# NetManAIOps/ChatTS

Hardware: NVIDIA H100
Metric: decode_tokens_per_s (higher is better)
Workload: dtype bf16

## Files before the change

chatts_b200/_cabi.py:

```python
import ctypes as C
import os

import torch

_HERE = os.path.dirname(os.path.abspath(__file__))
LIB_PATH = os.path.join(_HERE, "lib", "libchatts_b200.so")

OK = 0
BF16, F16 = 0, 1
EPI_NONE, EPI_GELU, EPI_SWIGLU, EPI_PARTIAL_F32, EPI_RESIDUAL, EPI_SPLITK_F32, EPI_SWIGLU_IL = 0, 1, 2, 3, 4, 5, 6

SYMBOLS = [
    "cts_version", "cts_arch", "cts_ctx_create", "cts_ctx_destroy", "cts_last_error",
    "cts_ts_patch_count", "cts_ts_patchify", "cts_gemm", "cts_gemm_suggest_split",
    "cts_reduce_bias_act", "cts_reduce_residual_rmsnorm", "cts_reduce_swiglu", "cts_qkv_rope_cache",
    "cts_embed_gather", "cts_attn_prefill", "cts_attn_decode_workspace_floats", "cts_attn_decode",
    "cts_greedy_advance", "cts_ipc_alloc", "cts_ipc_open", "cts_ipc_close", "cts_ipc_free",
    "cts_peer_allreduce_residual_rmsnorm", "cts_peer_greedy_advance", "cts_decode_chain",
    "cts_attn_prefill_lse", "cts_attn_bwd", "cts_swiglu", "cts_swiglu_bwd", "cts_rmsnorm_bwd", "cts_qkv_rope_bwd",
    "cts_ce_loss_grad", "cts_gather_rows", "cts_lora_wgrad", "cts_adamw", "cts_grad_norm_ws_floats", "cts_grad_norm_clip",
    "cts_lora_pack",
    "cts_sample_advance", "cts_rmsnorm", "cts_lm_head", "cts_decoder_step_ws_floats", "cts_decoder_step", "cts_ts_encode", "cts_gemm_decode_fused",
    "cts_peer_ll_region_bytes", "cts_peer_allreduce_ll", "cts_trace_enable", "cts_ts_encode_fused_ok", "cts_ts_encode_fused",
    "cts_rep_penalty_mark", "cts_rep_penalty_apply", "cts_gemm_w4", "cts_gemm_w4_suggest_split", "cts_gemm_w4_mma", "cts_gemm_w4_mma_suggest_split",
]
FUSED_RESIDUAL, FUSED_SWIGLU, FUSED_QKV_ROPE = 0, 1, 2
PACK_DESC_LONGS = 12


class CtsError(RuntimeError):
    pass


class GemmArgs(C.Structure):
    _fields_ = [
        ("w", C.c_void_p), ("w2", C.c_void_p), ("x", C.c_void_p), ("bias", C.c_void_p),
        ("residual", C.c_void_p), ("out", C.c_void_p), ("row_map", C.c_void_p),
        ("n", C.c_longlong), ("k", C.c_longlong), ("t", C.c_longlong),
        ("w_ld", C.c_longlong), ("x_ld", C.c_longlong), ("out_ld", C.c_longlong),
        ("dtype", C.c_int), ("epilogue", C.c_int), ("split_k", C.c_int), ("reserved", C.c_int),
        ("splitk_ws", C.c_void_p), ("tile_counters", C.c_void_p),
        ("next_w", C.c_void_p), ("next_n", C.c_longlong), ("next_k", C.c_longlong), ("next_ld", C.c_longlong),
        ("next_split", C.c_int), ("next_reserved", C.c_int), ("next_prefetch_bytes", C.c_longlong),
    ]


class ChainArgs(C.Structure):
    _fields_ = (
        [(k, C.c_int) for k in ("t", "hidden", "inter", "nh", "nkv", "head_dim", "phase_begin", "phase_end", "norm5_has_partial",
                                "dtype")] + [("split", C.c_int * 4)] +
        [(k, C.c_void_p) for k in ("wo", "wgu", "wd", "wqkv", "ao", "h", "xn", "act", "ln_post", "ln_next")] + [("eps", C.c_float)] +
        [(k, C.c_void_p) for k in ("bqkv", "q_norm_w", "k_norm_w", "positions", "cos_tab", "sin_tab", "slot_map", "q_out", "k_cache",
                                   "v_cache")] + [("page_size", C.c_int)] + [(k, C.c_void_p) for k in ("ws", "ssq", "sync")])


class LayerWeights(C.Structure):
    _fields_ = [(k, C.c_void_p) for k in ("wqkv", "bqkv", "q_norm", "k_norm", "wo", "wgu", "wd", "ln1", "ln2", "k_cache", "v_cache")]
# ... 70 lines not shown
    lib.cts_reduce_residual_rmsnorm.argtypes = [vp, vp, i, vp, vp, vp, f, vp, ll, ll, i, vp]
    lib.cts_reduce_swiglu.argtypes = [vp, vp, i, ll, ll, vp, i, i, vp]
    lib.cts_qkv_rope_cache.argtypes = [vp, vp, i, i, vp, vp, vp, vp, vp, vp, vp, vp, vp, vp, ll, i, i, i, i, vp, vp, f, i, vp]
    lib.cts_embed_gather.argtypes = [vp, vp, vp, vp, ll, ll, ll, i, vp]
    lib.cts_attn_prefill.argtypes = [vp, vp, vp, vp, vp, i, i, ll, i, i, i, f, vp, i, vp]
    lib.cts_attn_decode_workspace_floats.argtypes = [i, i, i, i]
    lib.cts_attn_decode_workspace_floats.restype = ll
    lib.cts_attn_decode.argtypes = [vp, vp, vp, vp, i, vp, i, vp, i, i, i, i, i, f, i, vp, vp, i, vp]
    lib.cts_greedy_advance.argtypes = [vp, vp, ll, i, vp, i, vp, vp, vp, vp, vp, vp, i, i, i, vp]
    lib.cts_ipc_alloc.argtypes = [vp, ll, C.POINTER(vp), C.c_char_p]
    lib.cts_ipc_open.argtypes = [vp, C.c_char_p, C.POINTER(vp)]
    lib.cts_ipc_close.argtypes = [vp, vp]
    lib.cts_ipc_free.argtypes = [vp, vp]
    lib.cts_peer_allreduce_residual_rmsnorm.argtypes = [vp, vp, i, vp, vp, vp, i, i, i, vp, vp, vp, f, vp, ll, ll, i, vp]
    lib.cts_peer_ll_region_bytes.argtypes = [i, i, ll]
    lib.cts_peer_ll_region_bytes.restype = ll
    lib.cts_peer_allreduce_ll.argtypes = [vp, vp, i, vp, ll, vp, i, i, i, vp, vp, vp, f, vp, ll, ll, i, vp]
    lib.cts_peer_allreduce_ll.restype = i
    lib.cts_trace_enable.argtypes = [vp, vp]
    lib.cts_gemm_w4.argtypes = [vp, C.POINTER(GemmW4Args), vp]
    lib.cts_gemm_w4_suggest_split.argtypes = [vp, ll, ll]
    lib.cts_gemm_w4_mma.argtypes = [vp, C.POINTER(GemmW4fArgs), vp]
    lib.cts_gemm_w4_mma_suggest_split.argtypes = [vp, ll, ll, ll]
    lib.cts_rep_penalty_mark.argtypes = [vp, vp, vp, i, vp, i, ll, vp]
    lib.cts_rep_penalty_apply.argtypes = [vp, vp, ll, ll, i, vp, i, f, i, vp]
    lib.cts_ts_encode_fused_ok.argtypes = [C.POINTER(TsEncodeArgs)]
    lib.cts_ts_encode_fused.argtypes = [vp, C.POINTER(TsEncodeArgs), vp]
    lib.cts_decode_chain.argtypes = [vp, C.POINTER(ChainArgs), vp]
    lib.cts_decode_chain.restype = i
    lib.cts_peer_greedy_advance.argtypes = [vp, vp, ll, i, i, i, vp, vp, vp, i, vp, i, vp, vp, vp, vp, vp, vp, i, i, i, vp]
    lib.cts_peer_greedy_advance.restype = i
    lib.cts_gemm_decode_fused.argtypes = [vp, C.POINTER(FusedGemmArgs), vp]
    lib.cts_gemm_decode_fused.restype = i
    lib.cts_ts_encode.argtypes = [vp, C.POINTER(TsEncodeArgs), vp]
    lib.cts_ts_encode.restype = i
    lib.cts_rmsnorm.argtypes = [vp, vp, vp, f, vp, ll, ll, i, vp]
    lib.cts_lm_head.argtypes = [vp, vp, vp, vp, ll, ll, ll, i, vp]
    lib.cts_decoder_step_ws_floats.argtypes = [C.POINTER(DecoderStepArgs)]
    lib.cts_decoder_step_ws_floats.restype = ll
    lib.cts_decoder_step.argtypes = [vp, C.POINTER(DecoderStepArgs), vp]
    for name in ("cts_rmsnorm", "cts_lm_head", "cts_decoder_step"):
        getattr(lib, name).restype = i
    lib.cts_sample_advance.argtypes = [vp, vp, ll, i, f, i, f, C.c_ulonglong, vp, i, vp, vp, vp, vp, vp, vp, i, i, i, vp]
    lib.cts_sample_advance.restype = i
    lib.cts_attn_prefill_lse.argtypes = [vp, vp, vp, vp, vp, i, i, ll, i, i, i, f, vp, vp, i, vp]
    lib.cts_attn_bwd.argtypes = [vp, vp, vp, vp, vp, vp, vp, vp, i, i, ll, i, i, i, f, vp, vp, vp, vp, i, vp]
    lib.cts_swiglu.argtypes = [vp, vp, ll, ll, i, vp, i, vp]
    lib.cts_swiglu_bwd.argtypes = [vp, vp, vp, ll, ll, i, vp, i, vp]
    lib.cts_rmsnorm_bwd.argtypes = [vp, vp, vp, vp, f, vp, vp, ll, ll, i, vp]
    lib.cts_qkv_rope_bwd.argtypes = [vp, vp, vp, vp, vp, vp, vp, vp, vp, vp, f, vp, ll, i, i, i, i, vp]
    lib.cts_ce_loss_grad.argtypes = [vp, vp, ll, vp, ll, ll, f, vp, vp, i, i, vp]
    lib.cts_gather_rows.argtypes = [vp, vp, vp, ll, ll, vp, i, vp]
    lib.cts_lora_wgrad.argtypes = [vp, vp, ll, ll, i, ll, vp, ll, ll, i, ll, f, vp, ll, ll, i, vp]
    lib.cts_adamw.argtypes = [vp, vp, vp, vp, vp, ll, f, f, f, f, f, i, vp, vp]
    lib.cts_grad_norm_ws_floats.argtypes = []
    lib.cts_grad_norm_ws_floats.restype = ll
    lib.cts_grad_norm_clip.argtypes = [vp, vp, ll, f, vp, vp, vp]
    lib.cts_lora_pack.argtypes = [vp, vp, vp, i, ll, vp, i, vp]
    for name in ("cts_attn_prefill_lse", "cts_attn_bwd", "cts_swiglu", "cts_swiglu_bwd", "cts_rmsnorm_bwd", "cts_qkv_rope_bwd",
                 "cts_ce_loss_grad", "cts_gather_rows", "cts_lora_wgrad", "cts_adamw", "cts_grad_norm_clip", "cts_lora_pack"):
        getattr(lib, name).restype = i
    for name in ("cts_ipc_alloc", "cts_ipc_open", "cts_ipc_close", "cts_ipc_free", "cts_peer_allreduce_residual_rmsnorm"):
        getattr(lib, name).restype = i
    for name in ("cts_ts_patch_count", "cts_ts_patchify", "cts_gemm", "cts_gemm_suggest_split", "cts_reduce_bias_act",
                 "cts_reduce_residual_rmsnorm", "cts_reduce_swiglu", "cts_qkv_rope_cache", "cts_embed_gather",
                 "cts_attn_prefill", "cts_attn_decode", "cts_greedy_advance", "cts_ctx_create"):
# ... 60 lines not shown
        self._trace = buf
        return buf

    def trace_end(self):
        torch.cuda.synchronize()
        self.lib.cts_trace_enable(self.h, None)
        buf, self._trace = self._trace, None
        n = min(int(buf[0]), int(buf[1]))
        return buf[2: 2 + 2 * n].view(n, 2).cpu().numpy()

    def ts_patch_count(self, x, num_features, patch_size):
        n = x.shape[0]
        row_len = x.numel() // max(n, 1)
        dev = x.device
        valid = torch.empty(n, dtype=torch.int32, device=dev)
        cnt = torch.empty(n, dtype=torch.int32, device=dev)
        off = torch.empty(n + 1, dtype=torch.int32, device=dev)
        mx = torch.empty(1, dtype=torch.int32, device=dev)
        self._chk(self.lib.cts_ts_patch_count(self.h, _p(x), dtype_code(x.dtype), n, row_len, num_features, patch_size,
                                              _p(valid), _p(cnt), _p(off), _p(mx), _stream()), 2)
        return valid, cnt, off, mx

    def ts_patchify(self, x, num_features, patch_size, mode, pos_table, emb_dim, max_seq_len, valid, off, mx,
                    max_patches, rows_out):
        n = x.shape[0]
        row_len = x.numel() // max(n, 1)
        self._chk(self.lib.cts_ts_patchify(self.h, _p(x), dtype_code(x.dtype), n, row_len, num_features, patch_size, mode,
                                           _p(pos_table), emb_dim, max_seq_len, _p(valid), _p(off), _p(mx), max_patches,
                                           _p(rows_out), rows_out.shape[1], _stream()))

    def suggest_split(self, n, k, t, dual=False):
        return int(self.lib.cts_gemm_suggest_split(self.h, n, k, t, int(dual)))

    def gemm(self, x, w, out, *, w2=None, bias=None, residual=None, row_map=None, epilogue=EPI_NONE, split_k=1, t=None,
             splitk_ws=None, tile_counters=None, next_w=None, next_split=1, next_bytes=0):
        a = GemmArgs()
        if next_w is not None and next_bytes > 0:
            a.next_w, a.next_n, a.next_k, a.next_ld = next_w.data_ptr(), next_w.shape[0], next_w.shape[1], next_w.stride(0)
            a.next_split, a.next_prefetch_bytes = int(next_split), int(next_bytes)
        a.w, a.w2, a.x = w.data_ptr(), (w2.data_ptr() if w2 is not None else None), x.data_ptr()
        a.bias = bias.data_ptr() if bias is not None else None
        a.residual = residual.data_ptr() if residual is not None else None
        a.out = out.data_ptr()
        a.row_map = row_map.data_ptr() if row_map is not None else None
        a.n, a.k = w.shape[0], w.shape[1]
        a.t = x.shape[0] if t is None else t
        a.w_ld, a.x_ld = w.stride(0), x.stride(0)
        a.out_ld = out.stride(-2) if epilogue not in (EPI_PARTIAL_F32, EPI_SPLITK_F32) else a.n
        a.splitk_ws = splitk_ws.data_ptr() if splitk_ws is not None else None
        a.tile_counters = tile_counters.data_ptr() if tile_counters is not None else None
        a.dtype, a.epilogue, a.split_k = dtype_code(x.dtype), epilogue, split_k
        self._chk(self.lib.cts_gemm(self.h, C.byref(a), _stream()))

    def gemm_w4(self, x, qw, scales, zeros, group_size, out, split_k, t=None):
        a = GemmW4Args()
        a.qw, a.scales, a.zeros, a.x, a.out = qw.data_ptr(), scales.data_ptr(), zeros.data_ptr(), x.data_ptr(), out.data_ptr()
        a.n, a.k = qw.shape[0], qw.shape[1] * 2
        a.t = x.shape[0] if t is None else t
        a.x_ld, a.group_size, a.split_k, a.dtype = x.stride(0), int(group_size), int(split_k), dtype_code(x.dtype)
        self._chk(self.lib.cts_gemm_w4(self.h, C.byref(a), _stream()))

    def gemm_w4_suggest_split(self, n, k):
        return int(self.lib.cts_gemm_w4_suggest_split(self.h, n, k))

    def gemm_w4_mma(self, x, qwf, szp, n, group_size, out, split_k, t=None):
        a = GemmW4fArgs()
# ... 305 lines not shown
```

chatts_b200/csrc/gemm_decode_fused.cu:

```cuda
#include <cooperative_groups.h>

#include <type_traits>

#include "common.cuh"

#ifndef CTS_DYN_SMEM
#define CTS_DYN_SMEM(name) extern __shared__ __align__(128) uint8_t name[]
#endif
#include "tensormap.cuh"
#include "trace.cuh"

namespace {

namespace cg = cooperative_groups;

constexpr int kBM = 128, kBK = 64, kThreads = 192, kMaxStages = 12;

struct FusedParams {
  long long n, k, t;
  int kb_total, split, stages, mode;
  const void* bias;
  void* h;
  void* act;
  const int* positions; const void* cos_tab; const void* sin_tab; const int* slot_map;
// ... 246 lines not shown
#pragma unroll
            for (int r = 0; r < 8; ++r)
              if (r < W) st_ll8(p.peer_region[r] + addr, wv, epoch);
          }
          if (p.ssq_out != nullptr) {
            const float ss = warp_sum(h0 * h0 + h1 * h1);
            if (lane == 0) red[ft >> 5] = ss;
            named_bar_sync(1, 128);
            if (ft < W)
              st_ll8(p.peer_region[ft] + sq_off + ((long long)t * gridDim.x + blockIdx.x) * 8, __float_as_uint(red[0] + red[1] + red[2] + red[3]),
                     epoch);
            named_bar_sync(1, 128);
          }
        }
      }
      for (int t = split; t < T_; t += S) {
        if (even) {
          const long long unit = ((long long)owner * Tmax + t) * hw + col;
          const uint8_t* src = mine + ag_off + (unit >> 2) * 16 + ((unit >> 1) & 1) * 8;
          uint2 v;
          unsigned spins = 0;
          while ((v = ld_ll8(src)).y != epoch)
            if (++spins > kPeerSpinLimit) peer_timeout("all-gather", me);
          *reinterpret_cast<uint32_t*>(hrow + (long long)t * p.n + f) = v.x;
        } else if (ft == 1 && p.ssq_out != nullptr) {
          const uint8_t* src = mine + sq_off + ((long long)t * gridDim.x + blockIdx.x) * 8;
          uint2 v;
          unsigned spins = 0;
          while ((v = ld_ll8(src)).y != epoch)
            if (++spins > kPeerSpinLimit) peer_timeout("statistics gather", me);
          p.ssq_out[(long long)t * gridDim.x + blockIdx.x] = __uint_as_float(v.x);
        }
      }
    } else
    for (int tb = split; tb < T_; tb += kGroup * S)
    for (int u = 0; u < kGroup; ++u) {
      if (u == 0) {
#pragma unroll
        for (int u2 = 0; u2 < kGroup; ++u2) {
          const int t2 = tb + u2 * S;
          float a2 = 0.f;
          if (t2 < T_)
            for (int s2 = 0; s2 < S; ++s2) a2 += *cluster.map_shared_rank(&part_s[t2 * kBM + ft], s2);
          accs[u2] = a2;
        }
      }
      const int t = tb + u * S;
      if (t >= T_) break;
      const float acc = accs[u];
      if (mode == CTS_FUSED_RESIDUAL) {
        float r = 0.f;
        if (f_ok) {
          T* hp = reinterpret_cast<T*>(p.h) + (long long)t * p.n + f;
          r = rnd<T>(DT<T>::to_f(*hp) + rnd<T>(acc));
          *hp = DT<T>::from_f(r);
        }
        if (p.ssq_out != nullptr) {
          const float ss = warp_sum(r * r);
          if (lane == 0) red[ft >> 5] = ss;
          named_bar_sync(1, 128);
          if (ft == 0) p.ssq_out[(long long)t * gridDim.x + blockIdx.x] = red[0] + red[1] + red[2] + red[3];
          named_bar_sync(1, 128);
        }
      } else if (mode == CTS_FUSED_SWIGLU) {
        if (ft >= 64) xch[ft - 64] = rnd<T>(acc);
        named_bar_sync(1, 128);
        if (ft < 64 && f_ok) {
          const long long i = (long long)(f0 >> 1) + ft;
          reinterpret_cast<T*>(p.act)[(long long)t * (p.n >> 1) + i] = DT<T>::from_f(rnd<T>(silu_f(rnd<T>(acc))) * xch[ft]);
        }
        named_bar_sync(1, 128);
      } else {
        const int d = p.d, half = d >> 1;
        const int head = (int)(f / d), i = (int)(f % d);
        const bool is_q = head < p.nh, is_k = !is_q && head < p.nh + p.nkv;
        float x = acc;
        if (p.bias != nullptr && f_ok) x += DT<T>::to_f(reinterpret_cast<const T*>(p.bias)[f]);
        x = rnd<T>(x);
        if (p.q_norm != nullptr || p.k_norm != nullptr) {
          float ss = warp_sum(f_ok ? x * x : 0.f);
          if (lane == 0) red[ft >> 5] = ss;
          named_bar_sync(1, 128);
          float tot;
          if (d == 128) tot = red[0] + red[1] + red[2] + red[3];
          else tot = (ft < 64) ? red[0] + red[1] : red[2] + red[3];
          named_bar_sync(1, 128);
          const T* nw = reinterpret_cast<const T*>(is_q ? p.q_norm : (is_k ? p.k_norm : nullptr));
          if (nw != nullptr && f_ok) {
            const float inv = 1.0f / sqrtf(tot / (float)d + p.eps);
            x = rnd<T>(DT<T>::to_f(nw[i]) * rnd<T>(x * inv));
          }
        }
        xch[ft] = x;
        named_bar_sync(1, 128);
        if (f_ok) {
          if (is_q || is_k) {
            const int pos = p.positions[t];
            const int ii = i < half ? i : i - half;
            const float c = DT<T>::to_f(reinterpret_cast<const T*>(p.cos_tab)[(long long)pos * half + ii]);
            const float sn = DT<T>::to_f(reinterpret_cast<const T*>(p.sin_tab)[(long long)pos * half + ii]);
            const float xp = xch[i < half ? ft + half : ft - half];
            x = i < half ? rnd<T>(rnd<T>(x * c) + rnd<T>(-xp * sn)) : rnd<T>(rnd<T>(x * c) + rnd<T>(xp * sn));
          }
          if (is_q) {
            reinterpret_cast<T*>(p.q_out)[(long long)t * p.nh * d + (long long)head * d + i] = DT<T>::from_f(x);
          } else {
            const int kvh = is_k ? head - p.nh : head - p.nh - p.nkv;
            T* cache = reinterpret_cast<T*>(is_k ? p.k_cache : p.v_cache);
            const int slot = p.slot_map ? p.slot_map[t] : -1;
            if (cache != nullptr && slot >= 0) {
              const long long page = slot / p.page_size, off = slot % p.page_size;
              cache[((page * p.nkv + kvh) * p.page_size + off) * d + i] = DT<T>::from_f(x);
            }
          }
        }
        named_bar_sync(1, 128);
      }
    }
  }
  cluster.sync();
  __syncthreads();
  if (threadIdx.x == 0) CTS_TRACE(CTS_TK_FUSED, 3);
  if (p.peer_region != nullptr && threadIdx.x == 0) {
    __threadfence();
    const int done = atomicAdd(&p.peer_state[1], 1) + 1;
    if (done == (int)(gridDim.x * gridDim.z)) {
      p.peer_state[1] = 0;
      p.peer_state[0] = p.peer_state[0] + 1;
      __threadfence();
    }
  }
}

template <typename T, int BN, bool NORM_IN>
int launch_fused(cts_ctx* ctx, const cts_fused_gemm_args* a, cudaStream_t stream) {
  const bool is_bf16 = a->dtype == CTS_BF16;
  CUtensorMap tm_w, tm_x;
  int rc = cts_make_tmap_2d(ctx, &tm_w, a->w, a->n, a->k, a->k, kBM, is_bf16);
  if (rc) return rc;
  if (NORM_IN) {
    tm_x = tm_w;
  } else {
    rc = cts_make_tmap_2d(ctx, &tm_x, a->x, a->t, a->k, a->k, BN, is_bf16);
    if (rc) return rc;
  }
  FusedParams p;
  memset(&p, 0, sizeof(p));
  p.n = a->n; p.k = a->k; p.t = a->t;
  p.kb_total = (int)cdiv_ll(a->k, kBK);
  p.split = a->split_k; p.mode = a->mode;
  p.bias = a->bias; p.h = a->h; p.act = a->act;
  p.positions = a->positions; p.cos_tab = a->cos_tab; p.sin_tab = a->sin_tab; p.slot_map = a->slot_map;
  p.q_out = a->q_out; p.k_cache = a->k_cache; p.v_cache = a->v_cache; p.q_norm = a->q_norm; p.k_norm = a->k_norm; p.eps = a->eps;
  p.nh = a->nh; p.nkv = a->nkv; p.d = a->head_dim; p.page_size = a->page_size;
  p.norm_h = a->norm_h; p.norm_w = a->norm_w; p.ssq_in = a->ssq_in; p.ssq_tiles = a->ssq_tiles; p.norm_eps = a->norm_eps;
  p.ssq_out = a->ssq_out;
  p.peer_region = (uint8_t* const*)a->peer_regions; p.peer_state = a->peer_state;
  p.peer_rank = a->peer_rank; p.peer_world = a->peer_world; p.peer_max_tokens = a->peer_max_tokens;
  constexpr int kStage = kBM * kBK * 2 + BN * kBK * 2;
  int stages = ctx->decode_stages * 1024 / kStage;
  if (stages > kMaxStages) stages = kMaxStages;
  if (stages < 2) stages = 2;
  while ((size_t)stages * kStage < (size_t)BN * kBM * 4) ++stages;
  p.stages = stages;
  const size_t smem = (size_t)stages * kStage + 1024;
  auto kern = gemm_decode_fused_kernel<T, BN, NORM_IN>;
  CTS_CUDA(ctx, cudaFuncSetAttribute(kern, cudaFuncAttributeMaxDynamicSharedMemorySize, (int)smem));
  cudaLaunchConfig_t cfg = {};
  cfg.gridDim = dim3((unsigned)cdiv_ll(a->n, kBM), 1, (unsigned)a->split_k);
  cfg.blockDim = dim3(kThreads);
  cfg.dynamicSmemBytes = smem;
  cfg.stream = stream;
  cudaLaunchAttribute attr[2];
  attr[0].id = cudaLaunchAttributeProgrammaticStreamSerialization;
  attr[0].val.programmaticStreamSerializationAllowed = 1;
  attr[1].id = cudaLaunchAttributeClusterDimension;
  attr[1].val.clusterDim.x = 1;
  attr[1].val.clusterDim.y = 1;
  attr[1].val.clusterDim.z = (unsigned)a->split_k;
  cfg.attrs = attr;
  cfg.numAttrs = 2;
  CTS_CUDA(ctx, cudaLaunchKernelEx(&cfg, kern, tm_w, tm_x, p));
  return CTS_OK;
}

}

extern "C" int cts_gemm_decode_fused(cts_ctx* ctx, const cts_fused_gemm_args* a, void* stream) {
  if (!ctx) return CTS_ERR_BAD_ARG;
  CTS_CHECK_ARG(ctx, a != nullptr && a->w, "null args / w");
  CTS_CHECK_ARG(ctx, a->n > 0 && a->k > 0 && a->t > 0 && a->t <= 32, "n, k > 0 and 1 <= t <= 32 (decode-sized step)");
  CTS_CHECK_ARG(ctx, a->dtype == CTS_BF16 || a->dtype == CTS_F16, "dtype");
  CTS_CHECK_ARG(ctx, a->split_k >= 1 && a->split_k <= 8, "1 <= split_k <= 8 (portable cluster size)");
  CTS_CHECK_ARG(ctx, a->split_k <= cdiv_ll(a->k, kBK), "split_k exceeds the number of 64-wide K blocks");
  CTS_CHECK_ARG(ctx, a->mode >= CTS_FUSED_RESIDUAL && a->mode <= CTS_FUSED_QKV_ROPE, "mode");
  if (a->mode == CTS_FUSED_RESIDUAL) CTS_CHECK_ARG(ctx, a->h != nullptr, "CTS_FUSED_RESIDUAL needs h");
  if (a->mode == CTS_FUSED_SWIGLU) CTS_CHECK_ARG(ctx, a->act != nullptr && a->n % 128 == 0, "CTS_FUSED_SWIGLU needs act and n % 128 == 0");
  if (a->mode == CTS_FUSED_QKV_ROPE) {
    CTS_CHECK_ARG(ctx, a->positions && a->cos_tab && a->sin_tab && a->q_out, "CTS_FUSED_QKV_ROPE needs positions, cos/sin tables, q_out");
    CTS_CHECK_ARG(ctx, (a->head_dim == 64 || a->head_dim == 128) && a->nh > 0 && a->nkv > 0 &&
                           a->n == (long long)(a->nh + 2 * a->nkv) * a->head_dim, "head_dim 64 or 128, n = (nh + 2 nkv) * head_dim");
    CTS_CHECK_ARG(ctx, a->page_size > 0 || a->k_cache == nullptr, "page_size");
  }
  if (a->peer_regions != nullptr) {
    CTS_CHECK_ARG(ctx, a->mode == CTS_FUSED_RESIDUAL && a->peer_state != nullptr, "the in-kernel all-reduce belongs to CTS_FUSED_RESIDUAL and needs peer_state");
    CTS_CHECK_ARG(ctx, a->peer_world >= 2 && a->peer_world <= 8 && a->peer_rank >= 0 && a->peer_rank < a->peer_world, "peer_world in 2..8, peer_rank");
    CTS_CHECK_ARG(ctx, a->n % (128LL * a->peer_world) == 0, "n must be a multiple of 128 * peer_world (a tile has one owner)");
    CTS_CHECK_ARG(ctx, a->t <= a->peer_max_tokens, "t exceeds peer_max_tokens");
    CTS_CHECK_ARG(ctx, a->peer_region_bytes >= (long long)a->peer_max_tokens * a->n * 12 + (long long)a->peer_max_tokens * (a->n / 128) * 8,
                  "symmetric region too small");
  }
  const bool norm_in = a->norm_h != nullptr;
  if (norm_in) {
    CTS_CHECK_ARG(ctx, a->norm_w && a->ssq_in && a->ssq_tiles > 0 && a->k % 8 == 0, "NORM_IN needs norm_w, ssq_in, ssq_tiles > 0 and k % 8 == 0");
  } else {
    CTS_CHECK_ARG(ctx, a->x != nullptr, "x is required unless norm_h is given");
  }
  cudaStream_t st = (cudaStream_t)stream;
#define FUSED_GO(TT)                                                                                              \
  if (norm_in) return a->t <= 16 ? launch_fused<TT, 16, true>(ctx, a, st) : launch_fused<TT, 32, true>(ctx, a, st); \
  return a->t <= 16 ? launch_fused<TT, 16, false>(ctx, a, st) : launch_fused<TT, 32, false>(ctx, a, st);
  if (a->dtype == CTS_BF16) { FUSED_GO(__nv_bfloat16) }
  FUSED_GO(__half)
#undef FUSED_GO
}

CTS_TRACE_SETTER(cts_trace_set_fused)
```

chatts_b200/model.py:

```python
import math
from dataclasses import dataclass

import numpy as np
import torch

from . import _cabi, layout
from .trace import span
from ._cabi import EPI_NONE, EPI_PARTIAL_F32, EPI_RESIDUAL, EPI_SWIGLU_IL
from .config import ChatTSConfig
from .ts_encoder import TimeSeriesEmbedding
from .weights import load_checkpoint, shard_tensor, synthetic_state_dict


@dataclass
class CausalLMOutput:
    logits: torch.Tensor


def rope_tables(cfg, n_pos, dtype, device):
    d = cfg.head_dim
    inv_freq = 1.0 / (float(cfg.rope_theta) ** (torch.arange(0, d, 2, dtype=torch.int64).to(torch.float32) / d))
    pos = torch.arange(n_pos, dtype=torch.float32)
    freqs = (inv_freq[:, None] @ pos[None, :]).transpose(0, 1)
    return freqs.cos().to(dtype).to(device).contiguous(), freqs.sin().to(dtype).to(device).contiguous()
# ... 12 lines not shown

    def release(self, pages):
        self.free.extend(reversed(pages))


class _Step:
    pass


class ChatTSForCausalLM:
    def __init__(self, config, state_dict, device="cuda", dtype=torch.bfloat16, tp_rank=0, tp_size=1,
                 max_batch=32, max_seq_len=2048, page_size=64, use_cuda_graph=True, comm=None,
                 use_peer_allreduce=True, graph_with_tp=True, use_chain=None, use_sample_kernel=None, use_native_step=None, use_fused_decode=None, use_peer_ll=None):
        if not torch.cuda.is_available():
            raise _cabi.CtsError("chatts_b200 needs an H100 (sm_90a) GPU; there is no CPU fallback")
        self.config, self.dtype = config, dtype
        self.device = torch.device(device if str(device) != "cuda" else f"cuda:{torch.cuda.current_device()}")
        self.tp_rank, self.tp_size, self.comm = tp_rank, tp_size, comm
        self.ctx = _cabi.get_context(self.device)
        cfg = config
        assert cfg.num_key_value_heads % tp_size == 0 and cfg.num_attention_heads % tp_size == 0
        self.nh, self.nkv, self.d = cfg.num_attention_heads // tp_size, cfg.num_key_value_heads // tp_size, cfg.head_dim
        self.H, self.I = cfg.hidden_size, cfg.intermediate_size // tp_size
        self.V = cfg.vocab_size // tp_size if tp_size > 1 else cfg.vocab_size
        self.L = cfg.num_hidden_layers
        self.eps = float(cfg.rms_norm_eps)
        self.page_size, self.max_batch, self.max_seq_len = page_size, max_batch, max_seq_len
        self.max_pages = (max_seq_len + page_size - 1) // page_size
        self.use_cuda_graph = use_cuda_graph
        self.graph_with_tp = graph_with_tp
        import os as _os
        self.use_chain = bool(int(_os.environ.get("CTS_DECODE_CHAIN", "0"))) if use_chain is None else bool(use_chain)
        self.use_native_step = bool(int(_os.environ.get("CTS_NATIVE_STEP", "0"))) if use_native_step is None else bool(use_native_step)
        self.use_fused_decode = int(_os.environ.get("CTS_DECODE_FUSED", "0")) if use_fused_decode is None else int(use_fused_decode)
        self.use_peer_ll = (_os.environ.get("CTS_PEER_LL", "1") == "1") if use_peer_ll is None else bool(use_peer_ll)
        self.tp_prefill_exchange = _os.environ.get("CTS_TP_PREFILL_EXCHANGE", "rs_ag")
        self._nccl = False
        if tp_size > 1 and torch.distributed.is_available() and torch.distributed.is_initialized():
            try:
                self._nccl = str(torch.distributed.get_backend(comm)) == "nccl"
            except Exception:
                self._nccl = False
        self.use_sample_kernel = bool(int(_os.environ.get("CTS_SAMPLE_KERNEL", "1"))) if use_sample_kernel is None else bool(use_sample_kernel)
        self.next_prefetch_bytes = int(float(_os.environ.get("CTS_NEXT_PREFETCH_MB", "0")) * (1 << 20))
        self.w4 = None
        self._load(state_dict)
        n_pos = min(cfg.max_position_embeddings, max(self.max_pages * page_size, 16))
        self.cos, self.sin = rope_tables(cfg, n_pos, dtype, self.device)
        self.n_pos = n_pos
        num_pages = max_batch * self.max_pages
        self.kv = torch.zeros(self.L, 2, num_pages, self.nkv, page_size, self.d, device=self.device, dtype=dtype)
        self.pool = PagePool(num_pages)
        self._steps = {}
        self.peer, self.peer_tokens = None, 0
        if tp_size > 1 and use_peer_allreduce:
            from .tp import PeerBuffers
            self.peer_tokens = max(max_batch, 64)
            self.peer = PeerBuffers(self.ctx, tp_rank, tp_size, self.peer_tokens, self.H, group=comm)

    def _load(self, sd):
        cfg, dev, dt = self.config, self.device, self.dtype

        def take(name):
            t = sd[name]
            t = shard_tensor(name, t, cfg, self.tp_rank, self.tp_size)
            return t.to(dev, dt).contiguous()

# ... 160 lines not shown
        g = torch.Generator(device=self.device).manual_seed(seed)
        packed = {}

        def make(n_out, n_in):
            qw = torch.randint(0, 256, (n_out, n_in // 2), generator=g, device=self.device, dtype=torch.uint8)
            sc = ((torch.rand(n_out, n_in // group_size, generator=g, device=self.device) * 0.5 + 0.75) * (0.02 * 3.46 / 7.5)).to(self.dtype)
            zp = torch.randint(7, 10, (n_out, n_in // group_size), generator=g, device=self.device, dtype=torch.uint8)
            return qw, sc, zp

        d, H, I = self.d, self.H, self.I
        for l in range(self.L):
            p = f"model.layers.{l}."
            parts = {}
            for name, (n_out, n_in) in (("self_attn.q_proj", (self.nh * d, H)), ("self_attn.k_proj", (self.nkv * d, H)), ("self_attn.v_proj", (self.nkv * d, H)),
                                        ("self_attn.o_proj", (H, self.nh * d)), ("mlp.gate_proj", (I, H)), ("mlp.up_proj", (I, H)), ("mlp.down_proj", (H, I))):
                t = make(n_out, n_in)
                packed[p + name] = t
                parts[name] = dequantize_w4(*t, group_size)
            self.wqkv[l].copy_(torch.cat([parts["self_attn.q_proj"], parts["self_attn.k_proj"], parts["self_attn.v_proj"]], 0))
            self.wo[l].copy_(parts["self_attn.o_proj"])
            gp, up = parts["mlp.gate_proj"], parts["mlp.up_proj"]
            self.wgu[l].copy_(torch.stack([gp.view(-1, 64, H), up.view(-1, 64, H)], 1).reshape(2 * I, H))
            self.wd[l].copy_(parts["mlp.down_proj"])
            del parts
        return self.attach_w4(packed, group_size)

    def _splits(self, T):
        c = self.ctx
        import os
        ov = os.environ.get("CTS_SPLITS")
        if ov and T <= 32:
            a = [int(v) for v in ov.split(",")]
            return dict(qkv=a[0], o=a[1], gu=a[2], d=a[3])
        return dict(qkv=c.suggest_split(self.wqkv[0].shape[0], self.H, T), o=c.suggest_split(self.H, self.nh * self.d, T),
                    gu=c.suggest_split(self.I, self.H, T, True), d=c.suggest_split(self.H, self.I, T))

    def _ws_floats(self, T, sp):
        return max(sp["qkv"] * T * self.wqkv[0].shape[0] if sp["qkv"] > 1 else 0, sp["o"] * T * self.H if sp["o"] > 1 else 0,
                   sp["gu"] * T * 2 * self.I if T <= 128 else 0, sp["d"] * T * self.H if sp["d"] > 1 else 0, 1)

    def _w4_splits(self, T):
        w4, c = self.w4, self.ctx
        if w4["splits"] is not None:
            return w4["splits"]
        return dict(qkv=c.gemm_w4_mma_suggest_split(self.wqkv[0].shape[0], self.H, T), o=c.gemm_w4_mma_suggest_split(self.H, self.nh * self.d, T),
                    gu=c.gemm_w4_mma_suggest_split(2 * self.I, self.H, T), d=c.gemm_w4_mma_suggest_split(self.H, self.I, T))

    def _layers(self, st, T, attend):
        c, sp, eps = self.ctx, st.splits, self.eps
        I, H = self.I, self.H
        c.reduce_residual_rmsnorm(None, 0, st.h, None, self.ln1[0], eps, st.xn, t=T)
        fused = self.use_fused_decode and T <= 32 and st.k_lin is None
        nb = self.next_prefetch_bytes if (T <= 32 and st.k_lin is None) else 0
        w4 = self.w4 if (self.w4 is not None and T <= 32 and st.k_lin is None and not fused) else None
        if w4 is not None:
            sp = self._w4_splits(T)

        def proj(kind, l, x, w, split, **kw):
            if w4 is not None and w4["kernel"] == "mma":
                qwf, szp, n_out = w4[kind][l]
                c.gemm_w4_mma(x, qwf, szp, n_out, w4["group_size"], st.ws, split, t=T)
            elif w4 is not None:
                qw, sc, zp = w4[kind][l]
                c.gemm_w4(x, qw, sc, zp, w4["group_size"], st.ws, split, t=T)
            else:
                c.gemm(x, w, st.ws, epilogue=EPI_PARTIAL_F32, split_k=split, t=T, **kw)

        def nxt(w, split):
            return dict(next_w=w, next_split=split, next_bytes=nb) if nb > 0 else {}
        for l in range(self.L):
            kc, vc = self.kv[l, 0], self.kv[l, 1]
            if fused:
                nw = self.ln1[l + 1] if l + 1 < self.L else self.final_norm
                tp_deep = self.tp_size > 1 and self.use_peer_ll and self.peer is not None and H % (128 * self.tp_size) == 0
                deep = self.use_fused_decode >= 2 and (self.tp_size == 1 or tp_deep)
                pr = [None, None]
                so, sd = min(sp["o"], 8), min(sp["d"], 8)
                if deep and self.tp_size > 1:
                    cap = max(1, 148 // max(1, H // 128))
                    so, sd = min(so, cap), min(sd, cap)
                    pr = [(self.peer.partials[w], self.peer.part_bytes, self.peer.state, self.tp_rank, self.tp_size, self.peer.max_batch) for w in (0, 1)]
                rope = dict(bias=self.bqkv[l], positions=st.positions, cos=self.cos, sin=self.sin, slot_map=st.slot_map, q_out=st.q, k_cache=kc,
                            v_cache=vc, q_norm=self.qn[l], k_norm=self.kn[l], eps=eps, nh=self.nh, nkv=self.nkv, head_dim=self.d,
                            page_size=self.page_size)
                if deep:
                    if l == 0:
                        c.gemm_decode_fused(st.xn, self.wqkv[l], _cabi.FUSED_QKV_ROPE, min(sp["qkv"], 8), T, **rope)
                    else:
                        c.gemm_decode_fused(None, self.wqkv[l], _cabi.FUSED_QKV_ROPE, min(sp["qkv"], 8), T, norm_h=st.h, norm_w=self.ln1[l],
                                            ssq_in=st.ssq_b, norm_eps=eps, **rope)
                    attend(l)
                    c.gemm_decode_fused(st.ao, self.wo[l], _cabi.FUSED_RESIDUAL, so, T, h=st.h, ssq_out=st.ssq_a, peer=pr[0])
                    c.gemm_decode_fused(None, self.wgu[l], _cabi.FUSED_SWIGLU, min(sp["gu"], 8), T, act=st.act, norm_h=st.h, norm_w=self.ln2[l],
                                        ssq_in=st.ssq_a, norm_eps=eps)
                    c.gemm_decode_fused(st.act, self.wd[l], _cabi.FUSED_RESIDUAL, sd, T, h=st.h, ssq_out=st.ssq_b, peer=pr[1])
                    if l + 1 == self.L:
                        c.reduce_residual_rmsnorm(None, 0, st.h, None, self.final_norm, eps, st.xn, t=T)
                    continue
                c.gemm_decode_fused(st.xn, self.wqkv[l], _cabi.FUSED_QKV_ROPE, min(sp["qkv"], 8), T, **rope)
                attend(l)
                if self.tp_size > 1:
                    self._tp_row_parallel(st, T, st.ao, self.wo[l], self.ln2[l], 0, sp["o"])
                else:
                    c.gemm_decode_fused(st.ao, self.wo[l], _cabi.FUSED_RESIDUAL, min(sp["o"], 8), T, h=st.h)
                    c.reduce_residual_rmsnorm(None, 0, st.h, None, self.ln2[l], eps, st.xn, t=T)
                c.gemm_decode_fused(st.xn, self.wgu[l], _cabi.FUSED_SWIGLU, min(sp["gu"], 8), T, act=st.act)
                if self.tp_size > 1:
                    self._tp_row_parallel(st, T, st.act, self.wd[l], nw, 1, sp["d"])
                else:
                    c.gemm_decode_fused(st.act, self.wd[l], _cabi.FUSED_RESIDUAL, min(sp["d"], 8), T, h=st.h)
                    c.reduce_residual_rmsnorm(None, 0, st.h, None, nw, eps, st.xn, t=T)
                continue
# ... 192 lines not shown
                raise ValueError(f"sequence of {n_tok} tokens exceeds the {self.n_pos} positions of the rotary table "
                                 f"(min(max_position_embeddings, max_seq_len))")
            need = (n_tok + self.page_size - 1) // self.page_size
            if need > self.max_pages:
                raise ValueError(f"sequence of {n_tok} tokens exceeds max_seq_len {self.max_seq_len}")
            needs.append(need)
        if sum(needs) > len(self.pool.free):
            raise RuntimeError(f"KV cache exhausted: need {sum(needs)} pages, {len(self.pool.free)} free of {self.pool.num_pages}")
        held = []
        try:
            for b, need in enumerate(needs):
                pg = self.pool.alloc(need)
                held += pg
                pt[b, :need] = pg
        except BaseException:
            self.pool.release(held)
            raise
        return pt, held

    def _decode_state(self, B, max_new):
        key = B
        st = self._steps.get(key)
        if st is not None and st.out_tokens.shape[1] >= max_new:
            return st
        dev = self.device
        st = self._alloc_step(B, decode=True)
        st.B = B
        st.cur_ids = torch.zeros(B, device=dev, dtype=torch.int32)
        st.seq_lens = torch.zeros(B, device=dev, dtype=torch.int32)
        st.page_table = torch.zeros(B, self.max_pages, device=dev, dtype=torch.int32)
        st.out_tokens = torch.zeros(B, max(max_new, 256), device=dev, dtype=torch.int32)
        st.step_ptr = torch.zeros(2, device=dev, dtype=torch.int32)
        st.logits = torch.empty(B, self.V, device=dev, dtype=self.dtype)
        per = max(1, (2 * 148) // max(1, B * self.nkv))
        max_tiles = max(1, (self.max_seq_len + 63) // 64)
        st.attn_splits = int(max(1, min(per, max_tiles, 32)))
        import os
        if os.environ.get("CTS_ATTN_SPLITS"):
            st.attn_splits = int(os.environ["CTS_ATTN_SPLITS"])
        st.attn_ws = torch.zeros(self.ctx.attn_decode_workspace_floats(B, self.nh, self.d, st.attn_splits), device=dev,
                                 dtype=torch.float32)
        st.ssq = torch.zeros(B * 8, device=dev, dtype=torch.float32)
        tiles_h = (self.H + 127) // 128
        st.ssq_a = torch.zeros(B, tiles_h, device=dev, dtype=torch.float32)
        st.ssq_b = torch.zeros(B, tiles_h, device=dev, dtype=torch.float32)
        st.chain_sync = torch.zeros(2, device=dev, dtype=torch.int32)
        st.graph = st.graph_nosample = None
        self._steps[key] = st
        return st

    def _native_ok(self, B):
        return self.use_native_step and self.tp_size == 1 and B <= 128 and not self._chain_ok(B) and self.w4 is None

    def _chain_ok(self, B):
        return (self.w4 is None and self.use_chain and self.tp_size == 1 and B <= 32 and self.H % 64 == 0 and self.H // 64 <= 192 and self.I % 64 == 0)

    def _decode_layers_chain(self, st, attend):
        c, B, sp = self.ctx, st.B, st.splits
        common = dict(t=B, hidden=self.H, inter=self.I, nh=self.nh, nkv=self.nkv, head_dim=self.d,
                      splits=(sp["o"], sp["gu"], sp["d"], sp["qkv"]), h=st.h, xn=st.xn, act=st.act, ws=st.ws, ssq=st.ssq,
                      sync=st.chain_sync, eps=self.eps, dtype=self.dtype, positions=st.positions, cos=self.cos, sin=self.sin,
                      slot_map=st.slot_map, q_out=st.q, page_size=self.page_size)
        c.decode_chain(phases=(5, 8), norm5_has_partial=0, ln_next=self.ln1[0], wqkv=self.wqkv[0], bqkv=self.bqkv[0],
                       q_norm_w=self.qn[0], k_norm_w=self.kn[0], k_cache=self.kv[0, 0], v_cache=self.kv[0, 1], **common)
        for l in range(self.L):
            attend(l)
            last = l == self.L - 1
# ... 208 lines not shown
```

include/chatts_b200.h:

```cpp
#ifndef CHATTS_B200_H
#define CHATTS_B200_H

#ifdef __cplusplus
extern "C" {
#endif

#define CTS_OK 0
#define CTS_ERR_BAD_ARG (-1)
#define CTS_ERR_UNSUPPORTED (-2)
#define CTS_ERR_CUDA (-3)
#define CTS_ERR_NCCL (-4)

#define CTS_BF16 0
#define CTS_F16 1

typedef struct cts_ctx cts_ctx;

int cts_version(void);
const char* cts_arch(void);

int cts_ctx_create(int device, cts_ctx** out);
void cts_ctx_destroy(cts_ctx* ctx);
const char* cts_last_error(const cts_ctx* ctx);

// ... 102 lines not shown
  int phase_begin, phase_end, norm5_has_partial, dtype;
  int split[4];
  const void* wo; const void* wgu; const void* wd; const void* wqkv;
  const void* ao;
  void* h; void* xn; void* act;
  const void* ln_post; const void* ln_next; float eps;
  const void* bqkv; const void* q_norm_w; const void* k_norm_w;
  const int* positions; const void* cos_tab; const void* sin_tab; const int* slot_map;
  void* q_out; void* k_cache; void* v_cache; int page_size;
  float* ws; float* ssq; int* sync;
} cts_chain_args;

int cts_decode_chain(cts_ctx* ctx, const cts_chain_args* args, void* stream);


#define CTS_FUSED_RESIDUAL 0
#define CTS_FUSED_SWIGLU 1
#define CTS_FUSED_QKV_ROPE 2
typedef struct {
  const void* w; const void* x;
  long long n, k, t;
  int dtype, mode, split_k, reserved;
  const void* bias;
  void* h;
  void* act;
  const int* positions; const void* cos_tab; const void* sin_tab; const int* slot_map;
  void* q_out; void* k_cache; void* v_cache; const void* q_norm; const void* k_norm;
  float eps; int nh, nkv, head_dim, page_size;
  const void* norm_h; const void* norm_w; const float* ssq_in; int ssq_tiles; float norm_eps;
  float* ssq_out;
  const void* peer_regions; int* peer_state; int peer_rank, peer_world, peer_max_tokens, peer_reserved; long long peer_region_bytes;
} cts_fused_gemm_args;
int cts_gemm_decode_fused(cts_ctx* ctx, const cts_fused_gemm_args* args, void* stream);

int cts_rmsnorm(cts_ctx* ctx, const void* x, const void* w, float eps, void* out, long long t, long long h, int dtype, void* stream);
int cts_lm_head(cts_ctx* ctx, const void* hidden, const void* w, void* logits, long long t, long long h, long long vocab, int dtype,
                void* stream);

typedef struct {
  const void* x; int dtype, n_series, row_len, num_features, patch_size, mode;
  const void* pos_table; int emb_dim, max_seq_len;
  int num_layers, hidden, in0;
  const void* const* weights;
  const void* const* biases;
  int* valid_len; int* patch_cnt; int* row_offset; int* max_valid;
  long long total_rows;
  void* rows_ws; void* act_ws[2]; float* splitk_ws; long long splitk_floats;
  void* out; long long out_ld; const int* row_map;
} cts_ts_encode_args;
int cts_ts_encode(cts_ctx* ctx, const cts_ts_encode_args* args, void* stream);

int cts_ts_encode_fused_ok(const cts_ts_encode_args* args);
int cts_ts_encode_fused(cts_ctx* ctx, const cts_ts_encode_args* args, void* stream);

typedef struct {
  const void* wqkv;
  const void* bqkv;
  const void* q_norm;
  const void* k_norm;
  const void* wo;
  const void* wgu;
  const void* wd;
  const void* ln1;
  const void* ln2;
  void* k_cache;
  void* v_cache;
// ... 88 lines not shown
```

Before: 2580.

## Enable fused decode GEMM by default with occupancy-aware split selection

Turns on the cluster-based fused decode GEMM by default for single-GPU CUDA runs with small batch (T<=4). Adds an occupancy query so the split-K cluster size is lowered until all clusters fit co-resident. The SwiGLU and residual epilogues are rewritten to batch distributed-shared-memory reductions, and the QKV/RoPE epilogue hoists the cos/sin and slot loads out of the per-token loop. Hardcoded SM counts become the queried device SM count. The risk is that the fused path or the smaller splits are slower than the previous unfused default for some shapes.

```diff
diff --git a/chatts_b200/_cabi.py b/chatts_b200/_cabi.py
--- a/chatts_b200/_cabi.py
+++ b/chatts_b200/_cabi.py
@@ -23,6 +23,7 @@
     "cts_sample_advance", "cts_rmsnorm", "cts_lm_head", "cts_decoder_step_ws_floats", "cts_decoder_step", "cts_ts_encode", "cts_gemm_decode_fused",
     "cts_peer_ll_region_bytes", "cts_peer_allreduce_ll", "cts_trace_enable", "cts_ts_encode_fused_ok", "cts_ts_encode_fused",
     "cts_rep_penalty_mark", "cts_rep_penalty_apply", "cts_gemm_w4", "cts_gemm_w4_suggest_split", "cts_gemm_w4_mma", "cts_gemm_w4_mma_suggest_split",
+    "cts_gemm_decode_fused_suggest_split", "cts_gemm_decode_fused_max_clusters",
 ]
 FUSED_RESIDUAL, FUSED_SWIGLU, FUSED_QKV_ROPE = 0, 1, 2
 PACK_DESC_LONGS = 12
@@ -159,6 +160,10 @@
     lib.cts_peer_greedy_advance.restype = i
     lib.cts_gemm_decode_fused.argtypes = [vp, C.POINTER(FusedGemmArgs), vp]
     lib.cts_gemm_decode_fused.restype = i
+    lib.cts_gemm_decode_fused_suggest_split.argtypes = [vp, ll, ll, ll, i, i]
+    lib.cts_gemm_decode_fused_suggest_split.restype = i
+    lib.cts_gemm_decode_fused_max_clusters.argtypes = [vp, ll, i, i]
+    lib.cts_gemm_decode_fused_max_clusters.restype = i
     lib.cts_ts_encode.argtypes = [vp, C.POINTER(TsEncodeArgs), vp]
     lib.cts_ts_encode.restype = i
     lib.cts_rmsnorm.argtypes = [vp, vp, vp, f, vp, ll, ll, i, vp]
@@ -285,6 +290,18 @@
     def suggest_split(self, n, k, t, dual=False):
         return int(self.lib.cts_gemm_suggest_split(self.h, n, k, t, int(dual)))
 
+    def fused_suggest_split(self, n, k, t, dtype, dual=False):
+        s = int(self.lib.cts_gemm_decode_fused_suggest_split(self.h, n, k, t, int(dual), dtype_code(dtype)))
+        if s < 1:
+            raise CtsError(f"chatts_b200 error {s}: {self.lib.cts_last_error(self.h).decode()}")
+        return s
+
+    def fused_max_clusters(self, t, split, dtype):
+        c = int(self.lib.cts_gemm_decode_fused_max_clusters(self.h, t, split, dtype_code(dtype)))
+        if c < 0:
+            raise CtsError(f"chatts_b200 error {c}: {self.lib.cts_last_error(self.h).decode()}")
+        return c
+
     def gemm(self, x, w, out, *, w2=None, bias=None, residual=None, row_map=None, epilogue=EPI_NONE, split_k=1, t=None,
              splitk_ws=None, tile_counters=None, next_w=None, next_split=1, next_bytes=0):
         a = GemmArgs()
diff --git a/chatts_b200/csrc/gemm_decode_fused.cu b/chatts_b200/csrc/gemm_decode_fused.cu
--- a/chatts_b200/csrc/gemm_decode_fused.cu
+++ b/chatts_b200/csrc/gemm_decode_fused.cu
@@ -302,50 +302,101 @@
           p.ssq_out[(long long)t * gridDim.x + blockIdx.x] = __uint_as_float(v.x);
         }
       }
+    } else if (mode == CTS_FUSED_SWIGLU) {
+      constexpr int kSw = 8;
+      const int j = ft & 63;
+      const long long i = (long long)(f0 >> 1) + j;
+      const bool j_ok = f0 + j < p.n;
+      T* act = reinterpret_cast<T*>(p.act);
+      for (int m0 = ft >> 6; split + m0 * S < T_; m0 += 2 * kSw) {
+        float g[kSw], u[kSw];
+#pragma unroll
+        for (int q = 0; q < kSw; ++q) {
+          const int t = split + (m0 + 2 * q) * S;
+          float a = 0.f, b = 0.f;
+          if (t < T_)
+            for (int s2 = 0; s2 < S; ++s2) {
+              a += *cluster.map_shared_rank(&part_s[t * kBM + j], s2);
+              b += *cluster.map_shared_rank(&part_s[t * kBM + 64 + j], s2);
+            }
+          g[q] = a;
+          u[q] = b;
+        }
+#pragma unroll
+        for (int q = 0; q < kSw; ++q) {
+          const int t = split + (m0 + 2 * q) * S;
+          if (t < T_ && j_ok) act[(long long)t * (p.n >> 1) + i] = DT<T>::from_f(rnd<T>(silu_f(rnd<T>(g[q]))) * rnd<T>(u[q]));
+        }
+      }
+    } else if (mode == CTS_FUSED_RESIDUAL) {
+      constexpr int kRes = 8;
+      T* hcol = reinterpret_cast<T*>(p.h) + f;
+      for (int tb = split; tb < T_; tb += kRes * S) {
+        float a[kRes], hv[kRes];
+#pragma unroll
+        for (int q = 0; q < kRes; ++q) {
+          const int t = tb + q * S;
+          float a2 = 0.f, h2 = 0.f;
+          if (t < T_) {
+            for (int s2 = 0; s2 < S; ++s2) a2 += *cluster.map_shared_rank(&part_s[t * kBM + ft], s2);
+            if (f_ok) h2 = DT<T>::to_f(hcol[(long long)t * p.n]);
+          }
+          a[q] = a2;
+          hv[q] = h2;
+        }
+#pragma unroll
+        for (int q = 0; q < kRes; ++q) {
+          const int t = tb + q * S;
+          if (t >= T_) break;
+          float r = 0.f;
+          if (f_ok) {
+            r = rnd<T>(hv[q] + rnd<T>(a[q]));
+            hcol[(long long)t * p.n] = DT<T>::from_f(r);
+          }
+          if (p.ssq_out != nullptr) {
+            const float ss = warp_sum(r * r);
+            if (lane == 0) red[ft >> 5] = ss;
+            named_bar_sync(1, 128);
+            if (ft == 0) p.ssq_out[(long long)t * gridDim.x + blockIdx.x] = red[0] + red[1] + red[2] + red[3];
+            named_bar_sync(1, 128);
+          }
+        }
+      }
     } else
-    for (int tb = split; tb < T_; tb += kGroup * S)
-    for (int u = 0; u < kGroup; ++u) {
-      if (u == 0) {
-#pragma unroll
-        for (int u2 = 0; u2 < kGroup; ++u2) {
-          const int t2 = tb + u2 * S;
-          float a2 = 0.f;
-          if (t2 < T_)
-            for (int s2 = 0; s2 < S; ++s2) a2 += *cluster.map_shared_rank(&part_s[t2 * kBM + ft], s2);
-          accs[u2] = a2;
-        }
-      }
-      const int t = tb + u * S;
-      if (t >= T_) break;
-      const float acc = accs[u];
-      if (mode == CTS_FUSED_RESIDUAL) {
-        float r = 0.f;
-        if (f_ok) {
-          T* hp = reinterpret_cast<T*>(p.h) + (long long)t * p.n + f;
-          r = rnd<T>(DT<T>::to_f(*hp) + rnd<T>(acc));
-          *hp = DT<T>::from_f(r);
-        }
-        if (p.ssq_out != nullptr) {
-          const float ss = warp_sum(r * r);
-          if (lane == 0) red[ft >> 5] = ss;
-          named_bar_sync(1, 128);
-          if (ft == 0) p.ssq_out[(long long)t * gridDim.x + blockIdx.x] = red[0] + red[1] + red[2] + red[3];
-          named_bar_sync(1, 128);
-        }
-      } else if (mode == CTS_FUSED_SWIGLU) {
-        if (ft >= 64) xch[ft - 64] = rnd<T>(acc);
-        named_bar_sync(1, 128);
-        if (ft < 64 && f_ok) {
-          const long long i = (long long)(f0 >> 1) + ft;
-          reinterpret_cast<T*>(p.act)[(long long)t * (p.n >> 1) + i] = DT<T>::from_f(rnd<T>(silu_f(rnd<T>(acc))) * xch[ft]);
-        }
-        named_bar_sync(1, 128);
-      } else {
-        const int d = p.d, half = d >> 1;
-        const int head = (int)(f / d), i = (int)(f % d);
-        const bool is_q = head < p.nh, is_k = !is_q && head < p.nh + p.nkv;
-        float x = acc;
-        if (p.bias != nullptr && f_ok) x += DT<T>::to_f(reinterpret_cast<const T*>(p.bias)[f]);
+    for (int tb = split; tb < T_; tb += kGroup * S) {
+      const int d = p.d, half = d >> 1;
+      const int head = (int)(f / d), i = (int)(f % d);
+      const int ii = i < half ? i : i - half;
+      const bool is_q = head < p.nh, is_k = !is_q && head < p.nh + p.nkv;
+      const bool has_bias = p.bias != nullptr && f_ok;
+      const float bias = has_bias ? DT<T>::to_f(reinterpret_cast<const T*>(p.bias)[f]) : 0.f;
+      float cs[kGroup], sn[kGroup];
+      int slot[kGroup];
+#pragma unroll
+      for (int u2 = 0; u2 < kGroup; ++u2) {
+        const int t2 = tb + u2 * S;
+        float a2 = 0.f, c2 = 0.f, s2v = 0.f;
+        int sl = -1;
+        if (t2 < T_) {
+          for (int s2 = 0; s2 < S; ++s2) a2 += *cluster.map_shared_rank(&part_s[t2 * kBM + ft], s2);
+          if (f_ok && (is_q || is_k)) {
+            const int pos = p.positions[t2];
+            c2 = DT<T>::to_f(reinterpret_cast<const T*>(p.cos_tab)[(long long)pos * half + ii]);
+            s2v = DT<T>::to_f(reinterpret_cast<const T*>(p.sin_tab)[(long long)pos * half + ii]);
+          }
+          if (!is_q && p.slot_map != nullptr) sl = p.slot_map[t2];
+        }
+        accs[u2] = a2;
+        cs[u2] = c2;
+        sn[u2] = s2v;
+        slot[u2] = sl;
+      }
+#pragma unroll
+      for (int u = 0; u < kGroup; ++u) {
+        const int t = tb + u * S;
+        if (t >= T_) break;
+        float x = accs[u];
+        if (has_bias) x += bias;
         x = rnd<T>(x);
         if (p.q_norm != nullptr || p.k_norm != nullptr) {
           float ss = warp_sum(f_ok ? x * x : 0.f);
@@ -365,21 +416,17 @@
         named_bar_sync(1, 128);
         if (f_ok) {
           if (is_q || is_k) {
-            const int pos = p.positions[t];
-            const int ii = i < half ? i : i - half;
-            const float c = DT<T>::to_f(reinterpret_cast<const T*>(p.cos_tab)[(long long)pos * half + ii]);
-            const float sn = DT<T>::to_f(reinterpret_cast<const T*>(p.sin_tab)[(long long)pos * half + ii]);
+            const float c = cs[u], s = sn[u];
             const float xp = xch[i < half ? ft + half : ft - half];
-            x = i < half ? rnd<T>(rnd<T>(x * c) + rnd<T>(-xp * sn)) : rnd<T>(rnd<T>(x * c) + rnd<T>(xp * sn));
+            x = i < half ? rnd<T>(rnd<T>(x * c) + rnd<T>(-xp * s)) : rnd<T>(rnd<T>(x * c) + rnd<T>(xp * s));
           }
           if (is_q) {
             reinterpret_cast<T*>(p.q_out)[(long long)t * p.nh * d + (long long)head * d + i] = DT<T>::from_f(x);
           } else {
             const int kvh = is_k ? head - p.nh : head - p.nh - p.nkv;
             T* cache = reinterpret_cast<T*>(is_k ? p.k_cache : p.v_cache);
-            const int slot = p.slot_map ? p.slot_map[t] : -1;
-            if (cache != nullptr && slot >= 0) {
-              const long long page = slot / p.page_size, off = slot % p.page_size;
+            if (cache != nullptr && slot[u] >= 0) {
+              const long long page = slot[u] / p.page_size, off = slot[u] % p.page_size;
               cache[((page * p.nkv + kvh) * p.page_size + off) * d + i] = DT<T>::from_f(x);
             }
           }
@@ -400,6 +447,42 @@
       __threadfence();
     }
   }
+}
+
+template <int BN>
+int fused_stages(const cts_ctx* ctx) {
+  constexpr int kStage = kBM * kBK * 2 + BN * kBK * 2;
+  int stages = ctx->decode_stages * 1024 / kStage;
+  if (stages > kMaxStages) stages = kMaxStages;
+  if (stages < 2) stages = 2;
+  while ((size_t)stages * kStage < (size_t)BN * kBM * 4) ++stages;
+  return stages;
+}
+template <int BN>
+size_t fused_smem(int stages) { return (size_t)stages * (kBM * kBK * 2 + BN * kBK * 2) + 1024; }
+
+template <typename T, int BN>
+int max_clusters(cts_ctx* ctx, int split, int* out) {
+  const size_t smem = fused_smem<BN>(fused_stages<BN>(ctx));
+  auto kern = gemm_decode_fused_kernel<T, BN, false>;
+  CTS_CUDA(ctx, cudaFuncSetAttribute(kern, cudaFuncAttributeMaxDynamicSharedMemorySize, (int)smem));
+  cudaLaunchConfig_t cfg = {};
+  cfg.gridDim = dim3(1, 1, (unsigned)split);
+  cfg.blockDim = dim3(kThreads);
+  cfg.dynamicSmemBytes = smem;
+  cudaLaunchAttribute attr[1];
+  attr[0].id = cudaLaunchAttributeClusterDimension;
+  attr[0].val.clusterDim.x = 1;
+  attr[0].val.clusterDim.y = 1;
+  attr[0].val.clusterDim.z = (unsigned)split;
+  cfg.attrs = attr;
+  cfg.numAttrs = 1;
+#ifdef CTS_HOST_SHIM
+  *out = 1 << 30;
+#else
+  CTS_CUDA(ctx, cudaOccupancyMaxActiveClusters(out, kern, &cfg));
+#endif
+  return CTS_OK;
 }
 
 template <typename T, int BN, bool NORM_IN>
@@ -427,13 +510,8 @@
   p.ssq_out = a->ssq_out;
   p.peer_region = (uint8_t* const*)a->peer_regions; p.peer_state = a->peer_state;
   p.peer_rank = a->peer_rank; p.peer_world = a->peer_world; p.peer_max_tokens = a->peer_max_tokens;
-  constexpr int kStage = kBM * kBK * 2 + BN * kBK * 2;
-  int stages = ctx->decode_stages * 1024 / kStage;
-  if (stages > kMaxStages) stages = kMaxStages;
-  if (stages < 2) stages = 2;
-  while ((size_t)stages * kStage < (size_t)BN * kBM * 4) ++stages;
-  p.stages = stages;
-  const size_t smem = (size_t)stages * kStage + 1024;
+  p.stages = fused_stages<BN>(ctx);
+  const size_t smem = fused_smem<BN>(p.stages);
   auto kern = gemm_decode_fused_kernel<T, BN, NORM_IN>;
   CTS_CUDA(ctx, cudaFuncSetAttribute(kern, cudaFuncAttributeMaxDynamicSharedMemorySize, (int)smem));
   cudaLaunchConfig_t cfg = {};
@@ -495,4 +573,29 @@
 #undef FUSED_GO
 }
 
+extern "C" int cts_gemm_decode_fused_max_clusters(cts_ctx* ctx, long long t, int split, int dtype) {
+  if (!ctx) return CTS_ERR_BAD_ARG;
+  CTS_CHECK_ARG(ctx, t > 0 && t <= 32 && split >= 1 && split <= 8, "1 <= t <= 32 and 1 <= split <= 8");
+  CTS_CHECK_ARG(ctx, dtype == CTS_BF16 || dtype == CTS_F16, "dtype");
+  int n = 0;
+  int rc;
+  if (dtype == CTS_BF16) rc = t <= 16 ? max_clusters<__nv_bfloat16, 16>(ctx, split, &n) : max_clusters<__nv_bfloat16, 32>(ctx, split, &n);
+  else rc = t <= 16 ? max_clusters<__half, 16>(ctx, split, &n) : max_clusters<__half, 32>(ctx, split, &n);
+  return rc != CTS_OK ? rc : n;
+}
+
+extern "C" int cts_gemm_decode_fused_suggest_split(cts_ctx* ctx, long long n, long long k, long long t, int dual, int dtype) {
+  if (!ctx) return CTS_ERR_BAD_ARG;
+  CTS_CHECK_ARG(ctx, n > 0 && k > 0 && t > 0 && t <= 32, "n, k > 0 and 1 <= t <= 32");
+  int s = cts_gemm_suggest_split(ctx, n, k, t, dual);
+  if (s > 8) s = 8;
+  const long long tiles = cdiv_ll(dual ? 2 * n : n, kBM);
+  for (; s > 1; --s) {
+    const int c = cts_gemm_decode_fused_max_clusters(ctx, t, s, dtype);
+    if (c < 0) return c;
+    if (c >= tiles) break;
+  }
+  return s;
+}
+
 CTS_TRACE_SETTER(cts_trace_set_fused)
diff --git a/chatts_b200/model.py b/chatts_b200/model.py
--- a/chatts_b200/model.py
+++ b/chatts_b200/model.py
@@ -68,7 +68,10 @@
         import os as _os
         self.use_chain = bool(int(_os.environ.get("CTS_DECODE_CHAIN", "0"))) if use_chain is None else bool(use_chain)
         self.use_native_step = bool(int(_os.environ.get("CTS_NATIVE_STEP", "0"))) if use_native_step is None else bool(use_native_step)
-        self.use_fused_decode = int(_os.environ.get("CTS_DECODE_FUSED", "0")) if use_fused_decode is None else int(use_fused_decode)
+        if use_fused_decode is None:
+            use_fused_decode = int(_os.environ.get("CTS_DECODE_FUSED", "1" if tp_size == 1 and self.device.type == "cuda" else "0"))
+        self.use_fused_decode = int(use_fused_decode)
+        self.sm_count = torch.cuda.get_device_properties(self.device).multi_processor_count if self.device.type == "cuda" else 132
         self.use_peer_ll = (_os.environ.get("CTS_PEER_LL", "1") == "1") if use_peer_ll is None else bool(use_peer_ll)
         self.tp_prefill_exchange = _os.environ.get("CTS_TP_PREFILL_EXCHANGE", "rs_ag")
         self._nccl = False
@@ -295,8 +298,15 @@
         if ov and T <= 32:
             a = [int(v) for v in ov.split(",")]
             return dict(qkv=a[0], o=a[1], gu=a[2], d=a[3])
+        if self.use_fused_decode and self.tp_size == 1 and T <= self._fused_max_t() and self.device.type == "cuda":
+            dt = self.dtype
+            return dict(qkv=c.fused_suggest_split(self.wqkv[0].shape[0], self.H, T, dt), o=c.fused_suggest_split(self.H, self.nh * self.d, T, dt),
+                        gu=c.fused_suggest_split(self.I, self.H, T, dt, True), d=c.fused_suggest_split(self.H, self.I, T, dt))
         return dict(qkv=c.suggest_split(self.wqkv[0].shape[0], self.H, T), o=c.suggest_split(self.H, self.nh * self.d, T),
                     gu=c.suggest_split(self.I, self.H, T, True), d=c.suggest_split(self.H, self.I, T))
+
+    def _fused_max_t(self):
+        return 32 if self.use_fused_decode >= 2 else 4
 
     def _ws_floats(self, T, sp):
         return max(sp["qkv"] * T * self.wqkv[0].shape[0] if sp["qkv"] > 1 else 0, sp["o"] * T * self.H if sp["o"] > 1 else 0,
@@ -313,7 +323,7 @@
         c, sp, eps = self.ctx, st.splits, self.eps
         I, H = self.I, self.H
         c.reduce_residual_rmsnorm(None, 0, st.h, None, self.ln1[0], eps, st.xn, t=T)
-        fused = self.use_fused_decode and T <= 32 and st.k_lin is None
+        fused = self.use_fused_decode and T <= self._fused_max_t() and st.k_lin is None and self.w4 is None
         nb = self.next_prefetch_bytes if (T <= 32 and st.k_lin is None) else 0
         w4 = self.w4 if (self.w4 is not None and T <= 32 and st.k_lin is None and not fused) else None
         if w4 is not None:
@@ -340,7 +350,7 @@
                 pr = [None, None]
                 so, sd = min(sp["o"], 8), min(sp["d"], 8)
                 if deep and self.tp_size > 1:
-                    cap = max(1, 148 // max(1, H // 128))
+                    cap = max(1, self.sm_count // max(1, H // 128))
                     so, sd = min(so, cap), min(sd, cap)
                     pr = [(self.peer.partials[w], self.peer.part_bytes, self.peer.state, self.tp_rank, self.tp_size, self.peer.max_batch) for w in (0, 1)]
                 rope = dict(bias=self.bqkv[l], positions=st.positions, cos=self.cos, sin=self.sin, slot_map=st.slot_map, q_out=st.q, k_cache=kc,
@@ -599,7 +609,7 @@
         st.out_tokens = torch.zeros(B, max(max_new, 256), device=dev, dtype=torch.int32)
         st.step_ptr = torch.zeros(2, device=dev, dtype=torch.int32)
         st.logits = torch.empty(B, self.V, device=dev, dtype=self.dtype)
-        per = max(1, (2 * 148) // max(1, B * self.nkv))
+        per = max(1, (2 * self.sm_count) // max(1, B * self.nkv))
         max_tiles = max(1, (self.max_seq_len + 63) // 64)
         st.attn_splits = int(max(1, min(per, max_tiles, 32)))
         import os
diff --git a/include/chatts_b200.h b/include/chatts_b200.h
--- a/include/chatts_b200.h
+++ b/include/chatts_b200.h
@@ -158,6 +158,8 @@
   const void* peer_regions; int* peer_state; int peer_rank, peer_world, peer_max_tokens, peer_reserved; long long peer_region_bytes;
 } cts_fused_gemm_args;
 int cts_gemm_decode_fused(cts_ctx* ctx, const cts_fused_gemm_args* args, void* stream);
+int cts_gemm_decode_fused_suggest_split(cts_ctx* ctx, long long n, long long k, long long t, int dual, int dtype);
+int cts_gemm_decode_fused_max_clusters(cts_ctx* ctx, long long t, int split, int dtype);
 
 int cts_rmsnorm(cts_ctx* ctx, const void* x, const void* w, float eps, void* out, long long t, long long h, int dtype, void* stream);
 int cts_lm_head(cts_ctx* ctx, const void* hidden, const void* w, void* logits, long long t, long long h, long long vocab, int dtype,
```

After: 2586 (median of 6 runs). Within noise of the previous version (+0.2%).
